# dfm/george

Measured on NVIDIA H100. Metric: gp.compute+log_likelihood N-points/sec, higher is better.
Workload: dtype f64

## Files before the change

### george_b200/csrc/hodlr.cu

```cuda
#include <algorithm>
#include <cmath>
#include <cstdlib>
#include <cstring>
#include <vector>

#include "common.cuh"
#include "hodlr_kernels.cuh"
#include "hodlr_lu.cuh"
#include "hodlr_aca2.cuh"
#include "hodlr_leaf.cuh"
#include "kernel_eval.cuh"

namespace bgp {
int upload_program(const DevProgram& P, DevBuf<DevProgram>& buf, cudaStream_t s);
int kmat_grad_contract_launch(const DevProgram* dprog, int nd, int np, const unsigned* which_dev, const double* x,
                              int64_t n, const double* M, int64_t ldm, const double* alpha, double ca, double cm,
                              double* g_dev, double* diag_dev, DevBuf<double>& scratch, cudaStream_t s);
int fill_identity_launch(double* A, int64_t n, cudaStream_t s);
int kmat_symmetric_launch_auto(const DevProgram& P, const DevProgram* dprog, const double* x, int64_t n,
                               const double* diag_add, double* out, int64_t ld, cudaStream_t s);
int kmat_general_launch_auto(const DevProgram& P, const DevProgram* dprog, const double* x1, int64_t n1, const double* x2,
                             int64_t n2, double* out, int64_t ld, cudaStream_t s);
int kmat_diagonal_launch(const DevProgram* dprog, const double* x1, const double* x2, int64_t n, double* out,
                         cudaStream_t s, int members = 1, int64_t ostride = 0);
int64_t predict_chunk_cols(int64_t n, int64_t multiple);
int predict_var_launch(const double* B, const double* W, int64_t ld, int64_t n, int64_t c, const double* kdiag,
                       double* var, DevBuf<double>& scratch, cudaStream_t s);
int predict_gemm_sub(const double* A, int64_t lda, const double* B, int64_t ldb, int64_t m, int64_t nn, int64_t K,
                     bool lower, double* C, int64_t ldc, DevBuf<double>& slices, DevBuf<GemmDesc>& descs, cudaStream_t s);
bool comm_ready();
int comm_rank();
int comm_world();
int comm_allreduce_sum_f64(double* buf, size_t count, cudaStream_t s);
int comm_allgather_f64(const double* send, double* recv, size_t count, cudaStream_t s);
}
using namespace bgp;

struct HNode {
  int start, size, half, is_leaf, parent, dir, depth;
  int slot;
  int rank = 0, draws = 0, fallback = 0;
  int owned = 1;
  int top = 0;
};

struct PanelSet {
  DevBuf<double> V, U;
  int64_t ld = 0, row_off = 0;
  int vcols = 0, ucols = 0;
  double* vbase() const { return V.p - row_off; }
  double* ubase() const { return U.p - row_off; }
};

struct LevelInfo {
  std::vector<int> nodes;
  int set = 1;
  int cap = 0, max_cap = 0, vcol = 0, r = 0, ucol = 0;
  int max_half = 0, grow = 0;
  int desc_off = 0;
};

struct AcaGraphKey {
  A2Args a;
  int nn, ncc, nrc, shape, grid;
};

struct bgp_hodlr {
  cudaStream_t sA = nullptr, sB = nullptr;
  cudaEvent_t ev[8] = {nullptr};
  int64_t n = 0;
  int ndim = 0;
  bgp_hodlr_opts_t opts;
  bool computed = false;
  double log_det = 0.0;
  DevProgram prog;

  std::vector<HNode> nodes;
  std::vector<int> leaves;
  std::vector<LevelInfo> levels;
  std::vector<int> piv_off;
  std::vector<int> h_piv_rows, h_piv_cols;
  int max_leaf = 0, rtot = 0, vcols = 0, cut_depth = 0;
  int64_t row0 = 0, nloc = 0;
  std::vector<int64_t> shard_row0, shard_rows;

  DevBuf<DevProgram> d_prog;
  DevBuf<double> d_x, d_yerr, d_diag, d_L, d_leaf_logdet, d_node_logdet, d_S, d_W, d_scalar, d_rhs;
  PanelSet top, loc;
  const PanelSet& pset(const LevelInfo& L) const { return L.set == 0 ? top : loc; }
  DevBuf<double> d_inv, d_gscratch;
  DevBuf<double> d_xsend, d_xrecv;
  DevBuf<unsigned> d_which;
  LuWorkspace lu_ws;
  DevBuf<GemmDesc> d_gram_desc, d_upd_desc;
  std::vector<NodeDesc> h_nodes;
  std::vector<int> cap_hint;
  int64_t cap_hint_n = -1;
  int cap_hint_min_size = -1;
  DevBuf<LeafDesc> d_leaves;
  DevBuf<AcaDesc> d_aca;
  DevBuf<AcaOut> d_aca_out;
  DevBuf<NodeDesc> d_nodes;
  DevBuf<PanelTile> d_ptiles;
  int small_limit = SS_MAX_N;
  bool leaf_cols_wide = false;
  DevBuf<int> d_idx, d_piv_rows, d_piv_cols, d_ticket, d_chain_done, d_ncols_by_depth;
  DevBuf<uint32_t> d_chain_state;
  DevBuf<A2Node> d_a2nodes;
  DevBuf<A2State> d_a2states;
  DevBuf<MT19937> d_a2rngs;
  DevBuf<A2EPart> d_epart;
  DevBuf<int> d_cand, d_cand_k, d_cand_words, d_cand_L, d_cand_next, d_cand_live, d_cchunk_node, d_rchunk_node, d_nactive;
  DevBuf<double> d_node_box;
  DevBuf<double2> d_cand_xu;
  DevBuf<unsigned long long> d_cmax, d_stats;
  DevBuf<int4> d_work;
  DevBuf<int> d_work_count, d_iter;
  AcaGraphKey aca_key;
  cudaGraph_t aca_graph = nullptr;
  cudaGraphExec_t aca_exec = nullptr;
  cudaStream_t sC = nullptr;
  bool profile = false;
  std::vector<cudaEvent_t> prof_events;
  double prof[12] = {0, 0, 0, 0, 0, 0, 0, 0, 0, 0, 0, 0};
  DevBuf<double> d_vpart, d_upart, d_vmax;
  int aca_iters = 0;
  size_t w_cap = 0;

  double t_ms[5] = {0, 0, 0, 0, 0};
  double work[6] = {0, 0, 0, 0, 0, 0};
};

static int ensure_streams(bgp_hodlr* h) {
  if (!h->sA) {
    BGP_CUDA(cudaStreamCreateWithFlags(&h->sA, cudaStreamNonBlocking));
    BGP_CUDA(cudaStreamCreateWithFlags(&h->sB, cudaStreamNonBlocking));
    for (int i = 0; i < 8; ++i) BGP_CUDA(cudaEventCreate(&h->ev[i]));
  }
  return BGP_OK;
}

static void build_tree(bgp_hodlr* h, int start, int size, int dir, int parent, int depth) {
  HNode nd;
  nd.start = start; nd.size = size; nd.half = size / 2; nd.dir = dir; nd.parent = parent; nd.depth = depth;
  nd.is_leaf = !(nd.half >= h->opts.min_size);
  nd.slot = 0;
  const int id = (int)h->nodes.size();
  h->nodes.push_back(nd);
  if (!nd.is_leaf) {
    build_tree(h, start, nd.half, 0, id, depth + 1);
    build_tree(h, start + nd.half, size - nd.half, 1, id, depth + 1);
  }
}

static int hodlr_solve_dev(bgp_hodlr* h, double* b, int64_t nrhs, int64_t ldb, cudaStream_t s, int part);
static int hodlr_exchange_finish(bgp_hodlr* h);
static int hodlr_finish_top_impl(bgp_hodlr* h, bool allreduce);

constexpr size_t LS_SMEM_MAX = 200 * 1024;
constexpr int LS_MAX_LEAF = (int)(LS_SMEM_MAX / sizeof(double));

static bool leaf_solve_fits(int max_leaf, int cols) { return sizeof(double) * (size_t)max_leaf * cols <= LS_SMEM_MAX; }

static void set_sweep_func_attrs() {
  static std::atomic<uint64_t> done{0};
  int dev = 0;
  cudaGetDevice(&dev);
  const uint64_t bit = dev < 64 ? (1ull << dev) : 0;
  if (bit && (done.load(std::memory_order_relaxed) & bit)) return;
  cudaFuncSetAttribute(leaf_solve_kernel<1>, cudaFuncAttributeMaxDynamicSharedMemorySize, (int)LS_SMEM_MAX);
  cudaFuncSetAttribute(leaf_solve_kernel<2>, cudaFuncAttributeMaxDynamicSharedMemorySize, (int)LS_SMEM_MAX);
  cudaFuncSetAttribute(leaf_solve_kernel<4>, cudaFuncAttributeMaxDynamicSharedMemorySize, (int)LS_SMEM_MAX);
  cudaFuncSetAttribute(leaf_solve_kernel<LS_COLS>, cudaFuncAttributeMaxDynamicSharedMemorySize, (int)LS_SMEM_MAX);
  cudaFuncSetAttribute(leaf_solve_kernel<LS_COLS_WIDE>, cudaFuncAttributeMaxDynamicSharedMemorySize, (int)LS_SMEM_MAX);
  cudaFuncSetAttribute(small_solve_kernel, cudaFuncAttributeMaxDynamicSharedMemorySize, 160 * 1024);
  done.fetch_or(bit, std::memory_order_relaxed);
}

template <int COLS>
static int leaf_solve_launch(bgp_hodlr* h, double* X, int64_t ldx, const int* ncols_by_depth, int ncols_fixed,
                             int max_cols, cudaStream_t s) {
  const int ngroups = (max_cols + COLS - 1) / COLS;
  const dim3 grid((unsigned)(h->leaves.size() * (size_t)ngroups));
  const size_t smem = sizeof(double) * (size_t)h->max_leaf * COLS;
  leaf_solve_kernel<COLS><<<grid, LS_THREADS, smem, s>>>(h->d_leaves.p, h->d_L.p, X, ldx, ncols_by_depth, ncols_fixed,
                                                         h->max_leaf, ngroups);
  BGP_LAUNCH_CHECK();
  return BGP_OK;
}

static int launch_leaf_solve(bgp_hodlr* h, double* X, int64_t ldx, const int* ncols_by_depth, int ncols_fixed,
                             int max_cols, cudaStream_t s) {
  const int nl = (int)h->leaves.size();
  if (nl == 0 || max_cols == 0) return BGP_OK;
  const int m = h->max_leaf;
  if (h->leaf_cols_wide && max_cols > LS_COLS && leaf_solve_fits(m, LS_COLS_WIDE))
    return leaf_solve_launch<LS_COLS_WIDE>(h, X, ldx, ncols_by_depth, ncols_fixed, max_cols, s);
  int cols = max_cols <= 1 ? 1 : max_cols <= 2 ? 2 : max_cols <= 4 ? 4 : LS_COLS;
  while (cols > 1 && !leaf_solve_fits(m, cols)) cols /= 2;
  if (!leaf_solve_fits(m, cols)) {
    set_error("leaf size %d too large for the leaf solve kernel (at most %d rows)", m, LS_MAX_LEAF);
    return BGP_ERR_INVALID;
  }
  switch (cols) {
    case LS_COLS: return leaf_solve_launch<LS_COLS>(h, X, ldx, ncols_by_depth, ncols_fixed, max_cols, s);
    case 4: return leaf_solve_launch<4>(h, X, ldx, ncols_by_depth, ncols_fixed, max_cols, s);
    case 2: return leaf_solve_launch<2>(h, X, ldx, ncols_by_depth, ncols_fixed, max_cols, s);
    default: return leaf_solve_launch<1>(h, X, ldx, ncols_by_depth, ncols_fixed, max_cols, s);
  }
}

static int launch_level_big(bgp_hodlr* h, const LevelInfo& L, double* X, int64_t ldx, int ncolsW, int own_off, int factor,
                            int col_lo, int col_hi, cudaStream_t s);

static int launch_level(bgp_hodlr* h, const LevelInfo& L, double* X, int64_t ldx, int ncolsW, int own_off, int factor,
                        int col_lo, int col_hi, cudaStream_t s) {
  const int nn = (int)L.nodes.size();
  if (nn == 0 || L.r == 0) {
    return BGP_OK;
  }
  const int r = L.r;
  const int64_t stride = (int64_t)2 * r * ncolsW;
  const size_t need = (size_t)nn * stride;
  if (need > h->w_cap) { set_error("internal: W workspace too small (%zu > %zu)", need, h->w_cap); return BGP_ERR_CUDA; }
  BGP_CUDA(cudaMemsetAsync(h->d_W.p, 0, sizeof(double) * need, s));
  if (2 * r > h->small_limit) return launch_level_big(h, L, X, ldx, ncolsW, own_off, factor, col_lo, col_hi, s);
  const NodeDesc* nd = h->d_nodes.p + L.desc_off;
  const int max_nh = L.max_half + 1;
  if (r <= GTS_MAX_R) {
    dim3 grid((max_nh + GTS_ROWS - 1) / GTS_ROWS, nn * 2, (ncolsW + GTS_TC - 1) / GTS_TC);
    const double* vb = h->pset(L).vbase();
    const int64_t ldv = h->pset(L).ld;
    if (r <= 2) gram_tn_small_kernel<2><<<grid, GTS_THREADS, 0, s>>>(nd, vb, ldv, X, ldx, ncolsW, h->d_W.p, stride);
    else if (r <= 4) gram_tn_small_kernel<4><<<grid, GTS_THREADS, 0, s>>>(nd, vb, ldv, X, ldx, ncolsW, h->d_W.p, stride);
    else gram_tn_small_kernel<GTS_MAX_R><<<grid, GTS_THREADS, 0, s>>>(nd, vb, ldv, X, ldx, ncolsW, h->d_W.p, stride);
    BGP_LAUNCH_CHECK();
  } else {
    dim3 grid((max_nh + GT_CHUNK - 1) / GT_CHUNK, nn * 2, (ncolsW + GT_TC - 1) / GT_TC);
    gram_tn_kernel<<<grid, GT_THREADS, 0, s>>>(nd, h->pset(L).vbase(), h->pset(L).ld, X, ldx, ncolsW, h->d_W.p, stride);
    BGP_LAUNCH_CHECK();
  }
  {
    const size_t sbytes = sizeof(double) * (size_t)(2 * r) * (2 * r);
    small_solve_kernel<<<nn, SS_THREADS, sbytes, s>>>(nd, h->d_W.p, stride, ncolsW, own_off, factor, h->d_S.p,
                                                      h->d_node_logdet.p, L.desc_off);
    BGP_LAUNCH_CHECK();
  }
  if (col_hi > col_lo) {
    dim3 grid((max_nh + UP_ROWS - 1) / UP_ROWS, nn * 2, (col_hi - col_lo + UP_TC - 1) / UP_TC);
    update_nn_kernel<<<grid, UP_THREADS, 0, s>>>(nd, h->pset(L).ubase(), h->pset(L).ld, X, ldx, col_lo, col_hi, h->d_W.p, stride, 0);
    BGP_LAUNCH_CHECK();
  }
  return BGP_OK;
}

static int launch_level_big(bgp_hodlr* h, const LevelInfo& L, double* X, int64_t ldx, int ncolsW, int own_off, int factor,
                            int col_lo, int col_hi, cudaStream_t s) {
  const int nn = (int)L.nodes.size();
  const int r = L.r, n2 = 2 * r;
  const int64_t stride = (int64_t)n2 * ncolsW;
  const int64_t ldv = h->pset(L).ld, ldu = h->pset(L).ld;
  double* W = h->d_W.p;
  constexpr int KCHUNK = 4096;
  std::vector<LuNode> lun(nn);
  std::vector<GemmDesc> gram, upd;
  int max_nh = 0;
  for (int b = 0; b < nn; ++b) {
    const HNode& nd = h->nodes[L.nodes[b]];
    const int64_t s_off = h->h_nodes[L.desc_off + b].s_off;
    lun[b].S = h->d_S.p + s_off;
    lun[b].piv = reinterpret_cast<int*>(lun[b].S + (int64_t)n2 * n2);
    lun[b].logdet = h->d_node_logdet.p + L.desc_off + b;
    double* Wn = W + (int64_t)b * stride;
    for (int hh = 0; hh < 2; ++hh) {
      const int rs = nd.start + (hh ? nd.half : 0), nh = hh ? (nd.size - nd.half) : nd.half;
      max_nh = std::max(max_nh, nh);
      for (int k0 = 0; k0 < nh; k0 += KCHUNK) {
        GemmDesc g;
        g.A = h->pset(L).vbase() + (int64_t)L.vcol * ldv + rs + k0; g.lda = ldv;
        g.B = X + rs + k0; g.ldb = ldx;
// ... 190 lines not shown
      BGP_CUDA(cudaGraphInstantiate(&h->aca_exec, h->aca_graph, 0));
      h->aca_key = key;
    }
    BGP_CUDA(cudaGraphLaunch(h->aca_exec, s));
    int it_host = 0, act2[2] = {0, 0};
    BGP_CUDA(cudaMemcpyAsync(&it_host, h->d_iter.p, sizeof(int), cudaMemcpyDeviceToHost, s));
    BGP_CUDA(cudaMemcpyAsync(act2, h->d_nactive.p, sizeof(int) * 2, cudaMemcpyDeviceToHost, s));
    BGP_CUDA(cudaStreamSynchronize(s));
    iters = it_host;
    g_launches.fetch_add((uint64_t)7 * (uint64_t)std::max(iters - 1, 0), std::memory_order_relaxed);
    if (act2[0] > 0) { set_error("ACA did not terminate"); return BGP_ERR_CUDA; }
  } else {
    while (active > 0) {
      for (int rep = 0; rep < 8; ++rep) {
        BGP_TRY(launch_iteration(s, 0, 0, h->profile ? iters : -1));
        iters++;
      }
      int act2[2] = {0, 0};
      BGP_CUDA(cudaMemcpyAsync(act2, h->d_nactive.p, sizeof(int) * 2, cudaMemcpyDeviceToHost, s));
      BGP_CUDA(cudaStreamSynchronize(s));
      active = act2[0];
      if (iters > (1 << 22)) { set_error("ACA did not terminate"); return BGP_ERR_CUDA; }
    }
  }
  h->aca_iters = iters;
  {
    unsigned long long st4[4] = {0, 0, 0, 0};
    BGP_CUDA(cudaMemcpyAsync(st4, h->d_stats.p, sizeof(st4), cudaMemcpyDeviceToHost, s));
    BGP_CUDA(cudaStreamSynchronize(s));
    h->prof[1] = iters; h->prof[2] = (double)st4[0]; h->prof[3] = (double)st4[1]; h->prof[4] = (double)st4[2];
    h->prof[5] = (double)st4[3];
    if (h->profile) {
      double tot[6] = {0, 0, 0, 0, 0, 0};
      for (int i = 0; i < iters; ++i)
        for (int k = 0; k < 6; ++k) {
          float ms = 0;
          cudaEventElapsedTime(&ms, h->prof_events[(size_t)7 * i + k], h->prof_events[(size_t)7 * i + k + 1]);
          tot[k] += ms;
        }
      h->prof[0] = tot[0];
      for (int k = 0; k < 6; ++k) h->prof[6 + k] = tot[k];
    }
  }
  if (h->opts.exhaust_mode == BGP_EXHAUST_DENSE) {
    a2_dense_fill_kernel<<<dim3(nn, 64), 256, 0, s>>>(a);
    BGP_LAUNCH_CHECK();
    a2_dense_rank_kernel<<<(nn + 127) / 128, 128, 0, s>>>(a);
    BGP_LAUNCH_CHECK();
  }
  std::vector<A2State> hs(nn);
  BGP_CUDA(cudaMemcpyAsync(hs.data(), h->d_a2states.p, sizeof(A2State) * nn, cudaMemcpyDeviceToHost, s));
  BGP_CUDA(cudaStreamSynchronize(s));
  for (int i = 0; i < nn; ++i) {
    AcaOut o;
    o.rank = hs[i].rank; o.draws = hs[i].draws; o.fallback = hs[i].fallback; o.status = hs[i].status;
    houts[descs[i].node] = o;
  }
  return BGP_OK;
}

static int hodlr_compute_dev_impl(bgp_hodlr* h, const bgp_kernel_spec_t* spec, const double* x_dev, int64_t n,
                                  int32_t ndim, const double* yerr_dev, const bgp_hodlr_opts_t* opts_in) {
  h->computed = false;
  BGP_TRY(require_device());
  BGP_TRY(ensure_streams(h));
  BGP_TRY(build_dev_program(spec, &h->prog));
  if (h->prog.ndim != ndim) { set_error("dimension mismatch: kernel ndim %d, input ndim %d", h->prog.ndim, ndim); return BGP_ERR_DIM; }
  if (ndim > ACA_MAX_NDIM) { set_error("HODLR supports at most %d input dimensions", ACA_MAX_NDIM); return BGP_ERR_INVALID; }
  if (n <= 0 || n > (int64_t)0x7fffffff) { set_error("invalid number of points %lld", (long long)n); return BGP_ERR_INVALID; }
  bgp_hodlr_opts_t o;
  if (opts_in) o = *opts_in; else bgp_hodlr_default_opts(&o);
  if (o.min_size < 1) { set_error("min_size must be >= 1"); return BGP_ERR_INVALID; }
  if (o.shard_count < 1) o.shard_count = 1;
  if (o.shard_count & (o.shard_count - 1)) { set_error("shard_count must be a power of two"); return BGP_ERR_INVALID; }
  if (o.shard_rank < 0 || o.shard_rank >= o.shard_count) { set_error("invalid shard_rank"); return BGP_ERR_INVALID; }
  if (o.shard_count > 1 && o.rng_mode == BGP_RNG_REFERENCE) { set_error("rng_mode=reference serialises the tree and cannot be sharded"); return BGP_ERR_INVALID; }
  h->opts = o;
  h->n = n;
  h->ndim = ndim;
  cudaStream_t sA = h->sA, sB = h->sB;
  set_sweep_func_attrs();
  h->small_limit = SS_MAX_N;
  if (const char* e = getenv("BGP_SMALL_RANK_LIMIT")) h->small_limit = std::min(SS_MAX_N, atoi(e));
  h->leaf_cols_wide = false;
  if (const char* e = getenv("BGP_LEAF_COLS")) h->leaf_cols_wide = atoi(e) > LS_COLS;

  h->nodes.clear(); h->leaves.clear(); h->levels.clear();
  h->nodes.reserve(2 * (size_t)(n / std::max(1, o.min_size)) + 8);
  build_tree(h, 0, (int)n, 0, -1, 0);
  int cut = 0;
  while ((1 << cut) < o.shard_count) cut++;
  h->cut_depth = cut;
  int max_depth = 0;
  for (auto& nd : h->nodes) max_depth = std::max(max_depth, nd.depth);
  h->row0 = 0; h->nloc = n;
  if (o.shard_count > 1) {
    int seen = 0; bool found = false;
    h->shard_row0.clear(); h->shard_rows.clear();
    for (size_t i = 0; i < h->nodes.size(); ++i) {
      HNode& nd = h->nodes[i];
      if (nd.depth == cut) {
        if (seen == o.shard_rank) { h->row0 = nd.start; h->nloc = nd.size; found = true; }
        h->shard_row0.push_back(nd.start); h->shard_rows.push_back(nd.size);
        seen++;
      }
    }
    if (!found || seen != o.shard_count) { set_error("tree too shallow to shard %d ways (N=%lld, min_size=%d)", o.shard_count, (long long)n, o.min_size); return BGP_ERR_INVALID; }
    for (auto& nd : h->nodes) {
      nd.top = nd.depth < cut;
      nd.owned = !nd.top && nd.start >= h->row0 && nd.start + nd.size <= h->row0 + h->nloc;
    }
  }
  h->levels.assign(max_depth + 1, LevelInfo());
  for (size_t i = 0; i < h->nodes.size(); ++i) {
    HNode& nd = h->nodes[i];
    if (nd.is_leaf) { if (nd.owned) { nd.slot = (int)h->leaves.size(); h->leaves.push_back((int)i); } continue; }
    if (!(nd.owned || nd.top)) continue;
    LevelInfo& L = h->levels[nd.depth];
    nd.slot = (int)L.nodes.size();
    L.nodes.push_back((int)i);
    L.max_half = std::max(L.max_half, nd.size - nd.half);
  }
  while (!h->levels.empty() && h->levels.back().nodes.empty()) h->levels.pop_back();
  const int nlev = (int)h->levels.size();
  for (int l = 0; l < nlev; ++l) h->levels[l].set = (o.shard_count > 1 && l < cut) ? 0 : 1;
  h->top.ld = n; h->top.row_off = 0;
  h->loc.ld = h->nloc; h->loc.row_off = h->row0;

  const int rcap0 = o.rank_capacity > 0 ? o.rank_capacity : 128;
  for (auto& L : h->levels) {
    int mh = 0;
    for (int id : L.nodes) mh = std::max(mh, h->nodes[id].half);
    L.max_cap = std::max(1, mh);
    L.cap = std::min(rcap0, L.max_cap);
  }
  if (o.rank_capacity <= 0 && h->cap_hint_n == n && h->cap_hint_min_size == o.min_size && (int)h->cap_hint.size() == nlev)
    for (int l = 0; l < nlev; ++l) h->levels[l].cap = std::min(h->levels[l].max_cap, std::max(h->levels[l].cap, h->cap_hint[l]));

  BGP_TRY(upload_program(h->prog, h->d_prog, sA));
  BGP_TRY(h->d_x.reserve((size_t)n * ndim, sA));
  BGP_TRY(h->d_diag.reserve((size_t)n, sA));
  if (x_dev != h->d_x.p) BGP_CUDA(cudaMemcpyAsync(h->d_x.p, x_dev, sizeof(double) * n * ndim, cudaMemcpyDeviceToDevice, sA));
  square_kernel<<<(unsigned)std::min<int64_t>((n + 255) / 256, 1184), 256, 0, sA>>>(yerr_dev, h->d_diag.p, n);
  BGP_LAUNCH_CHECK();
  BGP_CUDA(cudaEventRecord(h->ev[0], sA));

  const int nl = (int)h->leaves.size();
  std::vector<LeafDesc> hleaves(nl);
  int64_t loff = 0;
  h->max_leaf = 0;
  for (int i = 0; i < nl; ++i) {
    const HNode& nd = h->nodes[h->leaves[i]];
    hleaves[i].start = nd.start; hleaves[i].size = nd.size; hleaves[i].depth = nd.depth; hleaves[i]._pad = 0;
    hleaves[i].off = loff;
    loff += (int64_t)nd.size * nd.size;
    h->max_leaf = std::max(h->max_leaf, nd.size);
  }
  if (h->max_leaf > LS_MAX_LEAF) {
    set_error("leaf size %d too large: the leaf solve handles at most %d rows (N=%lld, min_size=%d); lower min_size",
              h->max_leaf, LS_MAX_LEAF, (long long)n, o.min_size);
    return BGP_ERR_INVALID;
  }
  BGP_TRY(h->d_leaves.reserve(std::max(nl, 1), sA));
  BGP_TRY(h->d_L.reserve((size_t)std::max<int64_t>(loff, 1), sA));
  BGP_TRY(h->d_leaf_logdet.reserve(std::max(nl, 1), sA));
  if (nl) {
    BGP_CUDA(cudaMemcpyAsync(h->d_leaves.p, hleaves.data(), sizeof(LeafDesc) * nl, cudaMemcpyHostToDevice, sA));
    const char* lf_env = getenv("BGP_LEAF_FACTOR");
// ... 716 lines not shown
```

### george_b200/csrc/hodlr_kernels.cuh

```cuda
#pragma once

#include <cooperative_groups.h>

#include "common.cuh"
#include "kernel_eval.cuh"

namespace bgp {

namespace cg = cooperative_groups;

struct MT19937 {
  uint32_t mt[624];
  int idx;
};
__device__ inline void mt_seed(MT19937& g, uint32_t s) {
  g.mt[0] = s;
  for (int i = 1; i < 624; ++i) g.mt[i] = 1812433253u * (g.mt[i - 1] ^ (g.mt[i - 1] >> 30)) + (uint32_t)i;
  g.idx = 624;
}
__device__ inline uint32_t mt_next(MT19937& g) {
  if (g.idx >= 624) {
    for (int i = 0; i < 624; ++i) {
      const uint32_t y = (g.mt[i] & 0x80000000u) | (g.mt[(i + 1) % 624] & 0x7fffffffu);
      g.mt[i] = g.mt[(i + 397) % 624] ^ (y >> 1) ^ ((y & 1u) ? 0x9908b0dfu : 0u);
// ... 71 lines not shown
      const double inv = 1.0 / d;
      __syncthreads();
      for (int i = k + 1 + threadIdx.x; i < nb; i += LEAF_THREADS) panel[i][k] *= inv;
      __syncthreads();
      for (int t = threadIdx.x; t < (nb - k - 1) * (nb - k - 1); t += LEAF_THREADS) {
        const int i = k + 1 + t % (nb - k - 1), j = k + 1 + t / (nb - k - 1);
        if (i >= j) panel[i][j] -= panel[i][k] * d * panel[j][k];
      }
      __syncthreads();
    }
    if (threadIdx.x < nb) {
      const double d = panel[threadIdx.x][threadIdx.x];
      dinv[threadIdx.x] = 1.0 / d;
      logdet += log(fabs(d));
    }
    for (int t = threadIdx.x; t < nb * nb; t += LEAF_THREADS) {
      const int i = t % nb, j = t / nb;
      if (i >= j) A[(int64_t)(k0 + j) * m + k0 + i] = panel[i][j];
    }
    __syncthreads();
    const int rem = m - k0 - nb;
    if (rem <= 0) break;
    for (int i = threadIdx.x; i < rem; i += LEAF_THREADS) {
      double* row = A + k0 + nb + i;
      double w[LEAF_NB];
#pragma unroll
      for (int j = 0; j < LEAF_NB; ++j) w[j] = (j < nb) ? row[(int64_t)(k0 + j) * m] : 0.0;
#pragma unroll
      for (int j = 0; j < LEAF_NB; ++j) {
        if (j < nb) {
          double s = w[j];
#pragma unroll
          for (int q = 0; q < j; ++q) s -= w[q] * panel[j][q];
          w[j] = s;
        }
      }
#pragma unroll
      for (int j = 0; j < LEAF_NB; ++j)
        if (j < nb) row[(int64_t)(k0 + j) * m] = w[j] * dinv[j];
    }
    __syncthreads();
    {
      const int tiles = (rem + 3) / 4;
      const double* Lp = A + (int64_t)k0 * m + k0 + nb;
      for (int t = threadIdx.x; t < tiles * tiles; t += LEAF_THREADS) {
        const int ti = t % tiles, tj = t / tiles;
        if (ti < tj) continue;
        double acc[4][4];
#pragma unroll
        for (int a = 0; a < 4; ++a)
#pragma unroll
          for (int b = 0; b < 4; ++b) acc[a][b] = 0.0;
        for (int q = 0; q < nb; ++q) {
          const double dq = panel[q][q];
          double li[4], lj[4];
#pragma unroll
          for (int a = 0; a < 4; ++a) {
            const int i = ti * 4 + a, j = tj * 4 + a;
            li[a] = (i < rem) ? Lp[(int64_t)q * m + i] : 0.0;
            lj[a] = (j < rem) ? Lp[(int64_t)q * m + j] * dq : 0.0;
          }
#pragma unroll
          for (int a = 0; a < 4; ++a)
#pragma unroll
            for (int b = 0; b < 4; ++b) acc[a][b] += li[a] * lj[b];
        }
#pragma unroll
        for (int b = 0; b < 4; ++b)
#pragma unroll
          for (int a = 0; a < 4; ++a) {
            const int i = ti * 4 + a, j = tj * 4 + b;
            if (i < rem && j < rem && i >= j) A[(int64_t)(k0 + nb + j) * m + k0 + nb + i] -= acc[a][b];
          }
      }
    }
    __syncthreads();
  }
  logdet = block_sum(logdet, red);
  if (threadIdx.x == 0) leaf_logdet[blockIdx.x] = logdet;
}

constexpr int LS_THREADS = 256;
constexpr int LS_COLS = 8;
constexpr int LS_COLS_WIDE = 32;
constexpr int LS_NB = 32;
constexpr int LS_BATCH = 4;

template <int COLS>
__global__ void __launch_bounds__(LS_THREADS, COLS <= LS_COLS ? 3 : 1) leaf_solve_kernel(const LeafDesc* __restrict__ leaves,
                                                                const double* __restrict__ Lbuf,
                                                                double* __restrict__ X, int64_t ldx,
                                                                const int* __restrict__ ncols_by_depth, int ncols_fixed,
                                                                int max_m, int ngroups) {
  extern __shared__ double xs[];
  __shared__ double sL[LS_NB][LS_NB + 1];
  const LeafDesc lf = leaves[blockIdx.x / ngroups];
  const int ncols = ncols_by_depth ? ncols_by_depth[lf.depth] : ncols_fixed;
  const int c0 = (blockIdx.x % ngroups) * COLS;
  if (c0 >= ncols) return;
  const int nc = min(COLS, ncols - c0);
  const int m = lf.size;
  const double* A = Lbuf + lf.off;
  const int lane = threadIdx.x & 31, warp = threadIdx.x >> 5;
  constexpr int NW = LS_THREADS / 32;
  for (int t = threadIdx.x; t < m * COLS; t += LS_THREADS) {
    const int i = t % m, c = t / m;
    xs[c * max_m + i] = (c < nc) ? X[(int64_t)(c0 + c) * ldx + lf.start + i] : 0.0;
  }
  for (int kb = 0; kb < m; kb += LS_NB) {
    const int nb = min(LS_NB, m - kb);
    __syncthreads();
    for (int t = threadIdx.x; t < LS_NB * LS_NB; t += LS_THREADS) {
      const int i = t % LS_NB, k = t / LS_NB;
      sL[i][k] = (i < nb && k < nb && i > k) ? A[(int64_t)(kb + k) * m + kb + i] : 0.0;
    }
    __syncthreads();
    for (int c = warp; c < nc; c += NW) {
      double y = (lane < nb) ? xs[c * max_m + kb + lane] : 0.0;
      for (int k = 0; k < nb; ++k) {
        const double yk = __shfl_sync(0xffffffffu, y, k);
        if (lane > k) y -= sL[lane][k] * yk;
      }
      if (lane < nb) xs[c * max_m + kb + lane] = y;
    }
    __syncthreads();
    const int r0 = kb + nb;
    for (int i = r0 + threadIdx.x; i < m; i += LS_THREADS) {
      double acc[COLS];
#pragma unroll
      for (int c = 0; c < COLS; ++c) acc[c] = 0.0;
      const double* Li = A + (int64_t)kb * m + i;
#pragma unroll 8
      for (int k = 0; k < nb; ++k) {
        const double l = Li[(int64_t)k * m];
#pragma unroll
        for (int c = 0; c < COLS; ++c) acc[c] += l * xs[c * max_m + kb + k];
      }
#pragma unroll
      for (int c = 0; c < COLS; ++c) if (c < nc) xs[c * max_m + i] -= acc[c];
    }
  }
  __syncthreads();
  for (int t = threadIdx.x; t < m * nc; t += LS_THREADS) {
    const int i = t % m, c = t / m;
    xs[c * max_m + i] /= A[(int64_t)i * m + i];
  }
  const int nblk = (m + LS_NB - 1) / LS_NB;
  for (int b = nblk - 1; b >= 0; --b) {
    const int kb = b * LS_NB;
    const int nb = min(LS_NB, m - kb);
    const int r0 = kb + nb;
    __syncthreads();
    for (int t = threadIdx.x; t < LS_NB * LS_NB; t += LS_THREADS) {
      const int i = t % LS_NB, k = t / LS_NB;
      sL[i][k] = (i < nb && k < nb && i > k) ? A[(int64_t)(kb + k) * m + kb + i] : 0.0;
    }
    for (int k = warp; k < nb; k += NW) {
      double acc[COLS];
#pragma unroll
      for (int c = 0; c < COLS; ++c) acc[c] = 0.0;
      const double* Lk = A + (int64_t)(kb + k) * m;
      for (int i0 = r0 + lane; i0 < m; i0 += 32 * LS_BATCH) {
        double l[LS_BATCH];
#pragma unroll
        for (int j = 0; j < LS_BATCH; ++j) l[j] = (i0 + 32 * j < m) ? Lk[i0 + 32 * j] : 0.0;
#pragma unroll
        for (int j = 0; j < LS_BATCH; ++j) {
          const int i = i0 + 32 * j;
          if (i < m) {
#pragma unroll
            for (int c = 0; c < COLS; ++c) acc[c] += l[j] * xs[c * max_m + i];
          }
// ... 646 lines not shown
```

### george_b200/csrc/hodlr_leaf.cuh

```cuda
#pragma once

#include "gemm_dmma.cuh"
#include "hodlr_kernels.cuh"

namespace bgp {

constexpr int LF_THREADS = 256;
constexpr int LF_NB = 32;
constexpr int LF_MAX_LEAF = 768;

__host__ __device__ inline int lf_panel_ld(int max_m) { return ((max_m + 15) / 16) * 16 + 4; }

template <int SHAPE>
__global__ void __launch_bounds__(LF_THREADS, 2) leaf_factor_kernel(const DevProgram* __restrict__ gprog,
                                                                    const double* __restrict__ x,
                                                                    const double* __restrict__ diag,
                                                                    const LeafDesc* __restrict__ leaves,
                                                                    double* __restrict__ Lbuf,
                                                                    double* __restrict__ leaf_logdet, int ldp) {
  extern __shared__ __align__(16) double lf_smem[];
  double* pn = lf_smem;
  double* dall = lf_smem + LF_NB * ldp;
  DevProgram* P = reinterpret_cast<DevProgram*>(lf_smem + (LF_NB + 1) * ldp);
  __shared__ double red[32];
// ... 57 lines not shown
          for (int b = 0; b < 4; ++b)
#pragma unroll
            for (int e = 0; e < 2; ++e) {
              const int c = b * 8 + 2 * lc + e;
              if (i < rem && c < nb && i >= c) pn[c * ldp + i] -= acc[a][b][e];
            }
        }
      }
      __syncthreads();
    }
    if (warp == 0) {
      double w[LF_NB];
#pragma unroll
      for (int j = 0; j < LF_NB; ++j) w[j] = (j <= lane && lane < nb) ? pn[j * ldp + lane] : 0.0;
#pragma unroll
      for (int k = 0; k < LF_NB; ++k) {
        if (k < nb) {
          const double d = __shfl_sync(0xffffffffu, w[k], k);
          const double l = (lane > k && lane < nb) ? w[k] / d : 0.0;
          if (lane > k) w[k] = l;
          const double ld = l * d;
#pragma unroll
          for (int j = k + 1; j < LF_NB; ++j) {
            const double lj = __shfl_sync(0xffffffffu, l, j);
            if (j <= lane) w[j] -= ld * lj;
          }
        }
      }
      if (lane < nb) {
        double* col = A + (int64_t)k0 * m + k0 + lane;
        double d = 0.0;
#pragma unroll
        for (int j = 0; j < LF_NB; ++j) {
          if (j < lane) { pn[j * ldp + lane] = w[j]; col[(int64_t)j * m] = w[j]; }
          if (j == lane) d = w[j];
        }
        col[(int64_t)lane * m] = d;
        dall[k0 + lane] = d;
        dinv[lane] = 1.0 / d;
        logdet += log(fabs(d));
      }
    }
    __syncthreads();
    const volatile double* l11 = pn;
    for (int i = LF_NB + threadIdx.x; i < rem; i += LF_THREADS) {
      double w[LF_NB];
#pragma unroll
      for (int j = 0; j < LF_NB; ++j) w[j] = pn[j * ldp + i];
#pragma unroll
      for (int j = 0; j < LF_NB; ++j) {
        double s = w[j];
#pragma unroll
        for (int q = 0; q < j; ++q) s -= w[q] * l11[q * ldp + j];
        w[j] = s;
      }
      double* row = A + (int64_t)k0 * m + k0 + i;
#pragma unroll
      for (int j = 0; j < LF_NB; ++j) row[(int64_t)j * m] = w[j] * dinv[j];
    }
    __syncthreads();
  }
  logdet = block_sum(logdet, red);
  if (threadIdx.x == 0) leaf_logdet[blockIdx.x] = logdet;
}

__host__ inline size_t lf_smem_bytes(int shape, int max_m) {
  return sizeof(double) * (size_t)(LF_NB + 1) * lf_panel_ld(max_m) + (shape == BGP_SHAPE_GENERIC ? sizeof(DevProgram) : 0);
}

template <int SHAPE>
inline void leaf_factor_launch_shape(int n_leaves, int max_m, cudaStream_t s, const DevProgram* prog, const double* x,
                                     const double* diag, const LeafDesc* leaves, double* L, double* leaf_logdet) {
  const size_t smem = lf_smem_bytes(SHAPE, max_m);
  cudaFuncSetAttribute(leaf_factor_kernel<SHAPE>, cudaFuncAttributeMaxDynamicSharedMemorySize, (int)smem);
  leaf_factor_kernel<SHAPE><<<n_leaves, LF_THREADS, smem, s>>>(prog, x, diag, leaves, L, leaf_logdet, lf_panel_ld(max_m));
}

inline void leaf_factor_launch(int shape, int n_leaves, int max_m, cudaStream_t s, const DevProgram* prog,
                               const double* x, const double* diag, const LeafDesc* leaves, double* L,
                               double* leaf_logdet) {
  BGP_SHAPE_SWITCH(shape, (leaf_factor_launch_shape<SHAPE>(n_leaves, max_m, s, prog, x, diag, leaves, L, leaf_logdet)));
}

}
```

Measured before the change: 21.84 million.

## Add DMMA tensor-core leaf solve kernel for wide right-hand-side blocks

```diff
diff --git a/george_b200/csrc/hodlr.cu b/george_b200/csrc/hodlr.cu
--- a/george_b200/csrc/hodlr.cu
+++ b/george_b200/csrc/hodlr.cu
@@ -103,7 +103,6 @@
   DevBuf<NodeDesc> d_nodes;
   DevBuf<PanelTile> d_ptiles;
   int small_limit = SS_MAX_N;
-  bool leaf_cols_wide = false;
   DevBuf<int> d_idx, d_piv_rows, d_piv_cols, d_ticket, d_chain_done, d_ncols_by_depth;
   DevBuf<uint32_t> d_chain_state;
   DevBuf<A2Node> d_a2nodes;
@@ -162,6 +161,8 @@
 
 static bool leaf_solve_fits(int max_leaf, int cols) { return sizeof(double) * (size_t)max_leaf * cols <= LS_SMEM_MAX; }
 
+constexpr int LSD_MIN_COLS = 8;
+
 static void set_sweep_func_attrs() {
   static std::atomic<uint64_t> done{0};
   int dev = 0;
@@ -172,7 +173,8 @@
   cudaFuncSetAttribute(leaf_solve_kernel<2>, cudaFuncAttributeMaxDynamicSharedMemorySize, (int)LS_SMEM_MAX);
   cudaFuncSetAttribute(leaf_solve_kernel<4>, cudaFuncAttributeMaxDynamicSharedMemorySize, (int)LS_SMEM_MAX);
   cudaFuncSetAttribute(leaf_solve_kernel<LS_COLS>, cudaFuncAttributeMaxDynamicSharedMemorySize, (int)LS_SMEM_MAX);
-  cudaFuncSetAttribute(leaf_solve_kernel<LS_COLS_WIDE>, cudaFuncAttributeMaxDynamicSharedMemorySize, (int)LS_SMEM_MAX);
+  cudaFuncSetAttribute(leaf_solve_dmma_kernel, cudaFuncAttributeMaxDynamicSharedMemorySize,
+                       (int)lsd_smem_bytes(LSD_MAX_LEAF));
   cudaFuncSetAttribute(small_solve_kernel, cudaFuncAttributeMaxDynamicSharedMemorySize, 160 * 1024);
   done.fetch_or(bit, std::memory_order_relaxed);
 }
@@ -194,8 +196,13 @@
   const int nl = (int)h->leaves.size();
   if (nl == 0 || max_cols == 0) return BGP_OK;
   const int m = h->max_leaf;
-  if (h->leaf_cols_wide && max_cols > LS_COLS && leaf_solve_fits(m, LS_COLS_WIDE))
-    return leaf_solve_launch<LS_COLS_WIDE>(h, X, ldx, ncols_by_depth, ncols_fixed, max_cols, s);
+  if (max_cols > LSD_MIN_COLS && m <= LSD_MAX_LEAF) {
+    const int ngroups = (max_cols + LSD_COLS - 1) / LSD_COLS;
+    leaf_solve_dmma_kernel<<<(unsigned)(h->leaves.size() * (size_t)ngroups), LSD_THREADS, lsd_smem_bytes(m), s>>>(
+        h->d_leaves.p, h->d_L.p, X, ldx, ncols_by_depth, ncols_fixed, m, ngroups);
+    BGP_LAUNCH_CHECK();
+    return BGP_OK;
+  }
   int cols = max_cols <= 1 ? 1 : max_cols <= 2 ? 2 : max_cols <= 4 ? 4 : LS_COLS;
   while (cols > 1 && !leaf_solve_fits(m, cols)) cols /= 2;
   if (!leaf_solve_fits(m, cols)) {
@@ -552,8 +559,6 @@
   set_sweep_func_attrs();
   h->small_limit = SS_MAX_N;
   if (const char* e = getenv("BGP_SMALL_RANK_LIMIT")) h->small_limit = std::min(SS_MAX_N, atoi(e));
-  h->leaf_cols_wide = false;
-  if (const char* e = getenv("BGP_LEAF_COLS")) h->leaf_cols_wide = atoi(e) > LS_COLS;
 
   h->nodes.clear(); h->leaves.clear(); h->levels.clear();
   h->nodes.reserve(2 * (size_t)(n / std::max(1, o.min_size)) + 8);
diff --git a/george_b200/csrc/hodlr_kernels.cuh b/george_b200/csrc/hodlr_kernels.cuh
--- a/george_b200/csrc/hodlr_kernels.cuh
+++ b/george_b200/csrc/hodlr_kernels.cuh
@@ -177,12 +177,11 @@
 
 constexpr int LS_THREADS = 256;
 constexpr int LS_COLS = 8;
-constexpr int LS_COLS_WIDE = 32;
 constexpr int LS_NB = 32;
 constexpr int LS_BATCH = 4;
 
 template <int COLS>
-__global__ void __launch_bounds__(LS_THREADS, COLS <= LS_COLS ? 3 : 1) leaf_solve_kernel(const LeafDesc* __restrict__ leaves,
+__global__ void __launch_bounds__(LS_THREADS, 3) leaf_solve_kernel(const LeafDesc* __restrict__ leaves,
                                                                 const double* __restrict__ Lbuf,
                                                                 double* __restrict__ X, int64_t ldx,
                                                                 const int* __restrict__ ncols_by_depth, int ncols_fixed,
diff --git a/george_b200/csrc/hodlr_leaf.cuh b/george_b200/csrc/hodlr_leaf.cuh
--- a/george_b200/csrc/hodlr_leaf.cuh
+++ b/george_b200/csrc/hodlr_leaf.cuh
@@ -163,4 +163,177 @@
   BGP_SHAPE_SWITCH(shape, (leaf_factor_launch_shape<SHAPE>(n_leaves, max_m, s, prog, x, diag, leaves, L, leaf_logdet)));
 }
 
-}
+constexpr int LSD_THREADS = 256;
+constexpr int LSD_COLS = 32;
+constexpr int LSD_NB = 32;
+constexpr int LSD_MAX_LEAF = 256;
+
+__host__ __device__ inline int lsd_x_ld(int max_m) { return ((max_m + 31) / 32) * 32 + 4; }
+__host__ __device__ inline int lsd_l_ld(int max_m) { return ((max_m + 15) / 16) * 16 + 4; }
+__host__ inline size_t lsd_smem_bytes(int max_m) {
+  return sizeof(double) * ((size_t)LSD_COLS * lsd_x_ld(max_m) + 2 * (size_t)LSD_NB * lsd_l_ld(max_m) +
+                           (size_t)LSD_NB * (LSD_NB + 1));
+}
+
+__device__ __forceinline__ void cp_async16_cg(void* smem, const void* gmem) {
+  asm volatile("cp.async.cg.shared.global [%0], [%1], 16;\n" ::"r"(smem_u32(smem)), "l"(gmem));
+}
+
+__device__ __forceinline__ void lsd_stage(double* st, int lds, const double* A, int m, int kb, int nb, bool v16) {
+  const int rows = m - kb;
+  if (v16) {
+    const int nch = rows >> 1;
+    for (int t = threadIdx.x; t < nb * nch; t += LSD_THREADS) {
+      const int k = t / nch, p = t - k * nch;
+      cp_async16_cg(st + k * lds + 2 * p, A + (int64_t)(kb + k) * m + kb + 2 * p);
+    }
+  } else {
+    for (int t = threadIdx.x; t < nb * rows; t += LSD_THREADS) {
+      const int k = t / rows, i = t - k * rows;
+      cp_async8(st + k * lds + i, A + (int64_t)(kb + k) * m + kb + i, true);
+    }
+  }
+}
+
+__global__ void __launch_bounds__(LSD_THREADS, 1) leaf_solve_dmma_kernel(const LeafDesc* __restrict__ leaves,
+                                                                         const double* __restrict__ Lbuf,
+                                                                         double* __restrict__ X, int64_t ldx,
+                                                                         const int* __restrict__ ncols_by_depth,
+                                                                         int ncols_fixed, int max_m, int ngroups) {
+  extern __shared__ __align__(16) double lsd_smem[];
+  const int ldX = lsd_x_ld(max_m), ldS = lsd_l_ld(max_m);
+  double* xs = lsd_smem;
+  double* stg = xs + LSD_COLS * ldX;
+  double(*sD)[LSD_NB + 1] = reinterpret_cast<double(*)[LSD_NB + 1]>(stg + 2 * LSD_NB * ldS);
+  const LeafDesc lf = leaves[blockIdx.x / ngroups];
+  const int ncols = ncols_by_depth ? ncols_by_depth[lf.depth] : ncols_fixed;
+  const int c0 = (blockIdx.x % ngroups) * LSD_COLS;
+  if (c0 >= ncols) return;
+  const int nc = min(LSD_COLS, ncols - c0);
+  const int m = lf.size;
+  const double* A = Lbuf + lf.off;
+  const bool v16 = (reinterpret_cast<uintptr_t>(A) & 15) == 0 && (m & 1) == 0;
+  const int lane = threadIdx.x & 31, warp = threadIdx.x >> 5;
+  const int lr = lane >> 2, lc = lane & 3;
+  const int nblk = (m + LSD_NB - 1) / LSD_NB, mr = nblk * LSD_NB;
+  const int nsteps = 2 * nblk;
+
+  lsd_stage(stg, ldS, A, m, 0, min(LSD_NB, m), v16);
+  cp_async_commit();
+  for (int t = threadIdx.x; t < mr * LSD_COLS; t += LSD_THREADS) {
+    const int i = t % mr, c = t / mr;
+    xs[c * ldX + i] = (c < nc && i < m) ? X[(int64_t)(c0 + c) * ldx + lf.start + i] : 0.0;
+  }
+  for (int s = 0; s < nsteps; ++s) {
+    const bool fwd = s < nblk;
+    const int kb = (fwd ? s : nsteps - 1 - s) * LSD_NB;
+    const int nb = min(LSD_NB, m - kb), R = m - kb - nb;
+    const double* st = stg + (s & 1) * LSD_NB * ldS;
+    cp_async_wait<0>();
+    __syncthreads();
+    if (s + 1 < nsteps) {
+      const int kn = (s + 1 < nblk ? s + 1 : nsteps - 2 - s) * LSD_NB;
+      lsd_stage(stg + ((s + 1) & 1) * LSD_NB * ldS, ldS, A, m, kn, min(LSD_NB, m - kn), v16);
+    }
+    cp_async_commit();
+    if (fwd) {
+      {
+        double l[LSD_NB], y[LSD_COLS / 8];
+#pragma unroll
+        for (int k = 0; k < LSD_NB; ++k) l[k] = (lane > k && lane < nb) ? st[k * ldS + lane] : 0.0;
+#pragma unroll
+        for (int j = 0; j < LSD_COLS / 8; ++j) y[j] = xs[(warp + 8 * j) * ldX + kb + lane];
+#pragma unroll
+        for (int k = 0; k < LSD_NB; ++k)
+#pragma unroll
+          for (int j = 0; j < LSD_COLS / 8; ++j) y[j] -= l[k] * __shfl_sync(0xffffffffu, y[j], k);
+        if (lane < nb)
+#pragma unroll
+          for (int j = 0; j < LSD_COLS / 8; ++j) xs[(warp + 8 * j) * ldX + kb + lane] = y[j];
+      }
+      __syncthreads();
+      if (R > 0) {
+        double bf[LSD_NB / 4][4];
+#pragma unroll
+        for (int kk = 0; kk < LSD_NB / 4; ++kk)
+#pragma unroll
+          for (int n = 0; n < 4; ++n) bf[kk][n] = xs[(n * 8 + lr) * ldX + kb + kk * 4 + lc];
+        for (int t = warp * 8; t < R; t += 64) {
+          double acc[4][2];
+#pragma unroll
+          for (int n = 0; n < 4; ++n) { acc[n][0] = 0.0; acc[n][1] = 0.0; }
+#pragma unroll
+          for (int kk = 0; kk < LSD_NB / 4; ++kk) {
+            const double af = st[(kk * 4 + lc) * ldS + LSD_NB + t + lr];
+#pragma unroll
+            for (int n = 0; n < 4; ++n) dmma884(acc[n][0], acc[n][1], af, bf[kk][n]);
+          }
+          const int i = kb + LSD_NB + t + lr;
+          if (i < m)
+#pragma unroll
+            for (int n = 0; n < 4; ++n)
+#pragma unroll
+              for (int e = 0; e < 2; ++e) xs[(n * 8 + 2 * lc + e) * ldX + i] -= acc[n][e];
+        }
+      }
+    } else {
+      for (int t = threadIdx.x; t < LSD_NB * LSD_NB; t += LSD_THREADS) {
+        const int i = t % LSD_NB, k = t / LSD_NB;
+        sD[i][k] = (i < nb && k < nb && i > k) ? st[k * ldS + i] : 0.0;
+      }
+      {
+        const int kt = (warp & 3) * 8, ct = (warp >> 2) * 16;
+        double acc[2][2][2];
+#pragma unroll
+        for (int h = 0; h < 2; ++h)
+#pragma unroll
+          for (int n = 0; n < 2; ++n) { acc[h][n][0] = 0.0; acc[h][n][1] = 0.0; }
+        const double* Ak = st + (kt + lr) * ldS + LSD_NB;
+        const double* B0 = xs + (ct + lr) * ldX + kb + LSD_NB;
+        const double* B1 = B0 + 8 * ldX;
+        for (int r0 = 0; r0 < R; r0 += 8) {
+#pragma unroll
+          for (int h = 0; h < 2; ++h) {
+            const int r = r0 + 4 * h + lc;
+            const double af = r < R ? Ak[r] : 0.0;
+            dmma884(acc[h][0][0], acc[h][0][1], af, B0[r]);
+            dmma884(acc[h][1][0], acc[h][1][1], af, B1[r]);
+          }
+        }
+        const int k = kt + lr;
+        if (k < nb) {
+          const double d = st[k * ldS + k];
+#pragma unroll
+          for (int n = 0; n < 2; ++n)
+#pragma unroll
+            for (int e = 0; e < 2; ++e) {
+              double* p = xs + (ct + n * 8 + 2 * lc + e) * ldX + kb + k;
+              *p = *p / d - (acc[0][n][e] + acc[1][n][e]);
+            }
+        }
+      }
+      __syncthreads();
+      {
+        double l[LSD_NB], y[LSD_COLS / 8];
+#pragma unroll
+        for (int i = 0; i < LSD_NB; ++i) l[i] = sD[i][lane];
+#pragma unroll
+        for (int j = 0; j < LSD_COLS / 8; ++j) y[j] = xs[(warp + 8 * j) * ldX + kb + lane];
+#pragma unroll
+        for (int i = LSD_NB - 1; i >= 0; --i)
+#pragma unroll
+          for (int j = 0; j < LSD_COLS / 8; ++j) y[j] -= l[i] * __shfl_sync(0xffffffffu, y[j], i);
+        if (lane < nb)
+#pragma unroll
+          for (int j = 0; j < LSD_COLS / 8; ++j) xs[(warp + 8 * j) * ldX + kb + lane] = y[j];
+      }
+    }
+  }
+  __syncthreads();
+  for (int t = threadIdx.x; t < m * nc; t += LSD_THREADS) {
+    const int i = t % m, c = t / m;
+    X[(int64_t)(c0 + c) * ldx + lf.start + i] = xs[c * ldX + i];
+  }
+}
+
+}
```

Result: faster. 24.00 million (median of 6 runs) (+9.9%).
